# X-PLUG/Youku-mPLUG

Hardware: NVIDIA H100
Metric: video-text samples/sec (pretrain 1.3B, 8f x 224^2) (higher is better)
Workload: dtype bf16

## Files before the change

include/ymp.h:

```cpp
#ifndef YMP_H_
#define YMP_H_

#include <stddef.h>
#include <stdint.h>

#ifdef __cplusplus
extern "C" {
#endif

#define YMP_OK 0
#define YMP_EINVAL (-1)
#define YMP_ECUDA (-2)
#define YMP_ENOSUP (-3)

const char* ymp_last_error(void);
int ymp_abi_version(void);
uint64_t ymp_launch_count(void);
int ymp_set_pdl(int on);

typedef struct ymp_dropout_spec {
  const uint64_t* rng;
  uint32_t site;
  float p;
} ymp_dropout_spec;
// ... 110 lines not shown
  const void* k;
  const void* v;
  void* o;
  float* lse;
  int32_t ldq, ldk, ldv, ldo;
  int32_t q_head_stride, k_head_stride, v_head_stride, o_head_stride;
  ymp_seqmap map_q, map_kv, map_o;
  int32_t n_seq, n_heads, head_dim, s_q, s_kv;
  int32_t mask;
  int32_t mask_block;
  int64_t total_rows;
  float scale;
  ymp_dropout_spec drop;
  const int32_t* s_kv_dev;
  const int32_t* kv_rows;
  int64_t kv_rows_ld;
} ymp_attn_args;
int ymp_attn_fwd(const ymp_attn_args* a, void* stream);

typedef struct ymp_attn_prefix_table_args {
  ymp_attn_args attn;
  const int32_t* n_prefix;
} ymp_attn_prefix_table_args;
int ymp_attn_fwd_prefix_table(const ymp_attn_prefix_table_args* a, void* stream);

typedef struct ymp_attn_prefix_kv_args {
  ymp_attn_prefix_table_args table;
  const void* k_cache;
  const void* v_cache;
  int32_t ld_cache;
  int32_t cache_head_stride;
  int32_t n0;
  int32_t _pad;
} ymp_attn_prefix_kv_args;
int ymp_attn_fwd_prefix_kv(const ymp_attn_prefix_kv_args* a, void* stream);

typedef struct ymp_attn_bwd_args {
  ymp_attn_args fwd;
  const void* dout;
  void* dq;
  void* dk;
  void* dv;
  float* delta_ws;
  int32_t lddo, lddq, lddk, lddv;
  int32_t do_head_stride, dq_head_stride, dk_head_stride, dv_head_stride;
  ymp_seqmap map_do, map_dq, map_dkv;
} ymp_attn_bwd_args;
int ymp_attn_bwd(const ymp_attn_bwd_args* a, void* stream);
#define YMP_ATTN_PATH_MMA_SYNC 0
#define YMP_ATTN_PATH_WGMMA 1
#define YMP_ATTN_PATH_SMALL 2
#define YMP_ATTN_PATH_DECODE 3
int ymp_attn_last_path(void);

typedef struct ymp_im2col_args {
  const void* video;
  void* out;
  int32_t B, C, T, H, W, P, ldo;
} ymp_im2col_args;
int ymp_im2col(const ymp_im2col_args* a, void* stream);

typedef struct ymp_clip_args {
  const void* frames;
  void* out;
  const void* lut;
  int32_t B, T, H, W, C;
} ymp_clip_args;
int ymp_clip_normalize(const ymp_clip_args* a, void* stream);

typedef struct ymp_dropout_args {
  const void* x;
  void* y;
  int32_t rows, cols, ldx, ldy;
  int32_t dtype;
  int64_t row0;
  ymp_dropout_spec drop;
} ymp_dropout_args;
int ymp_dropout(const ymp_dropout_args* a, void* stream);

typedef struct ymp_embed_args {
  const int64_t* ids;
  const void* table;
  const void* pos;
  void* out;
  int32_t B, L, S, row_offset, hidden, vocab, ldo;
  int32_t out_dtype;
} ymp_embed_args;
int ymp_embed_gather(const ymp_embed_args* a, void* stream);

typedef struct ymp_ce_args {
  const void* logits;
  const int64_t* labels;
  float* loss;
  float* lse;
  const float* grad_rows;
  void* dlogits;
  int32_t rows, V, ld;
} ymp_ce_args;
int ymp_ce_fwd(const ymp_ce_args* a, void* stream);
int ymp_ce_bwd(const ymp_ce_args* a, void* stream);

typedef struct ymp_colsum_args {
  const void* in;
  float* out;
  int32_t R, C, ld;
} ymp_colsum_args;
// ... 34 lines not shown
```

youku-mplug_b200/csrc/attention.cu:

```cuda
#include <math_constants.h>
#include <stdlib.h>

#include "common.h"
#include "philox.cuh"
#include "ptx.cuh"
#include "wgmma.cuh"

namespace ymp {

struct SeqMap {
  int seq_div, n_prefix, prefix_per_seq;
  long outer_stride, inner_stride, pos_stride, prefix_base, prefix_stride;
};
static SeqMap to_map(const ymp_seqmap& m) {
  SeqMap r;
  r.seq_div = m.seq_div > 0 ? m.seq_div : 1;
  r.n_prefix = m.n_prefix; r.prefix_per_seq = m.prefix_per_seq;
  r.outer_stride = m.outer_stride; r.inner_stride = m.inner_stride; r.pos_stride = m.pos_stride;
  r.prefix_base = m.prefix_base; r.prefix_stride = m.prefix_stride;
  return r;
}
struct RSeq {
  long base, pos_stride, prefix0;
  int n_prefix;
// ... 293 lines not shown
  for (int r = 0; r < 2; ++r) {
    l_i[r] += __shfl_xor_sync(0xffffffffu, l_i[r], 1);
    l_i[r] += __shfl_xor_sync(0xffffffffu, l_i[r], 2);
  }
#pragma unroll
  for (int r = 0; r < 2; ++r) {
    const int qi = row_lo + g + r * 8;
    if ((unsigned)qi >= (unsigned)sq) continue;
    const float inv = l_i[r] > 0.f ? 1.f / l_i[r] : 0.f;
    __nv_bfloat16* orow = p.o + rrow(mo, qi) * p.ldo + h * p.hso;
#pragma unroll
    for (int nb = 0; nb < DIO / 8; ++nb)
      *reinterpret_cast<uint32_t*>(orow + nb * 8 + t4 * 2) = pack_bf16(o_acc[nb][2 * r] * inv, o_acc[nb][2 * r + 1] * inv);
    if (p.lse && t4 == 0) p.lse[((size_t)s * p.n_heads + h) * p.s_q + qi] = m_i[r] * p.scale + logf(l_i[r]);
  }
}
template <int D, int DIO>
__device__ __forceinline__ void store_dq(const AttnKParams& p, const float (&dq_acc)[D / 8][4], int row_lo, int sq, int h,
                                         const RSeq& mdq, int g, int t4) {
#pragma unroll
  for (int r = 0; r < 2; ++r) {
    const int qi = row_lo + g + r * 8;
    if (qi >= sq) continue;
    __nv_bfloat16* dqrow = p.dq + rrow(mdq, qi) * p.lddq + h * p.hsdq;
#pragma unroll
    for (int nb = 0; nb < DIO / 8; ++nb)
      *reinterpret_cast<uint32_t*>(dqrow + nb * 8 + t4 * 2) = pack_bf16(dq_acc[nb][2 * r] * p.scale, dq_acc[nb][2 * r + 1] * p.scale);
  }
}
template <int D, int DIO>
__device__ __forceinline__ void store_dkdv(const AttnKParams& p, const float (&dk_acc)[D / 8][4],
                                           const float (&dv_acc)[D / 8][4], int row_lo, int skv, int h, const RSeq& mdkv,
                                           int g, int t4) {
#pragma unroll
  for (int r = 0; r < 2; ++r) {
    const int kvr = row_lo + g + r * 8;
    if (kvr >= skv) continue;
    const long row = rrow(mdkv, kvr);
    __nv_bfloat16* dkrow = p.dk + row * p.lddk + h * p.hsdk;
    __nv_bfloat16* dvrow = p.dv + row * p.lddv + h * p.hsdv;
#pragma unroll
    for (int nb = 0; nb < DIO / 8; ++nb) {
      *reinterpret_cast<uint32_t*>(dkrow + nb * 8 + t4 * 2) = pack_bf16(dk_acc[nb][2 * r] * p.scale, dk_acc[nb][2 * r + 1] * p.scale);
      *reinterpret_cast<uint32_t*>(dvrow + nb * 8 + t4 * 2) = pack_bf16(dv_acc[nb][2 * r], dv_acc[nb][2 * r + 1]);
    }
  }
}

enum TileLayout {
  PADDED,
  SWIZZLE_128B
};
template <TileLayout L, int D, int DIO, class M>
__device__ __forceinline__ void load_tile(void* dst, const M& m, int r0, int n_valid, const int* rows = nullptr) {
  constexpr int CH = D / 8;
#pragma unroll
  for (int it = 0; it < (64 * CH + 127) / 128; ++it) {
    const int idx = threadIdx.x + it * 128;
    if ((64 * CH) % 128 != 0 && idx >= 64 * CH) break;
    const int r = idx / CH, c = idx - r * CH;
    uint8_t* d = L == PADDED ? reinterpret_cast<uint8_t*>(static_cast<__nv_bfloat16*>(dst) + r * (D + 8) + c * 8)
                             : static_cast<uint8_t*>(dst) + (c >> 3) * 8192 + r * 128 + (((c & 7) ^ (r & 7)) << 4);
    if ((unsigned)(r0 + r) < (unsigned)n_valid && (DIO == D || c * 8 < DIO))
      cp_async16(d, mrow(m, rows ? __ldg(rows + r0 + r) : r0 + r) + c * 8);
    else *reinterpret_cast<uint4*>(d) = make_uint4(0, 0, 0, 0);
  }
}

template <int D, int DIO>
__global__ void __launch_bounds__(128) attn_fwd_kernel(const AttnKParams p) {
  constexpr int LDS = D + 8, KS = D / 16, TILE = 64 * LDS;
  extern __shared__ __align__(16) uint8_t smem_attn[];
  __nv_bfloat16* Qs = reinterpret_cast<__nv_bfloat16*>(smem_attn);
  __nv_bfloat16* KVs = Qs + TILE;
  const int warp = threadIdx.x >> 5, lane = threadIdx.x & 31;
  const int q0 = blockIdx.x * 64, h = blockIdx.y, s = blockIdx.z;
  const int g = lane >> 2, t4 = lane & 3;
  griddep_launch();
  griddep_wait();
  int sq, skv;
  eff_len(p, s, sq, skv);
  if (q0 >= sq) return;
  const int* table = p.kv_rows ? p.kv_rows + s * p.kv_rows_ld : nullptr;
  const RSeq mkv = table ? RSeq{0, 1, 0, 0} : resolve(p.mkv, s), mo = resolve(p.mo, s);
  const RMat Mq = rmat(p.q, resolve(p.mq, s), p.ldq, h * p.hsq);
  const RMat Mk = rmat(p.k, mkv, p.ldk, h * p.hsk), Mv = rmat(p.v, mkv, p.ldv, h * p.hsv);
  int kv_begin;
  const int ntiles = key_tiles<true>(p, q0, sq, skv, kv_begin);

  load_tile<PADDED, D, DIO>(Qs, Mq, q0, sq);
  load_tile<PADDED, D, DIO>(KVs, Mk, kv_begin, skv, table);
  load_tile<PADDED, D, DIO>(KVs + TILE, Mv, kv_begin, skv, table);
  cp_async_commit();

  uint32_t qf[KS][4];
  float o_acc[D / 8][4];
#pragma unroll
  for (int i = 0; i < D / 8; ++i) { o_acc[i][0] = o_acc[i][1] = o_acc[i][2] = o_acc[i][3] = 0.f; }
  float m_i[2] = {-CUDART_INF_F, -CUDART_INF_F}, l_i[2] = {0.f, 0.f};
  const bool warp_active = (q0 + warp * 16) < sq;
  DropState ds;
  if (p.has_drop) ds = drop_state(p.drop);
  const uint32_t drow0 = (uint32_t)(((long)s * p.n_heads + h) * p.s_q + q0 + warp * 16 + g);

  for (int t = 0; t < ntiles; ++t) {
    const int kv0 = kv_begin + t * 64;
    __nv_bfloat16* Ks = KVs + (t & 1) * 2 * TILE;
    __nv_bfloat16* Vs = Ks + TILE;
    if (t + 1 < ntiles) {
      __nv_bfloat16* Kn = KVs + ((t + 1) & 1) * 2 * TILE;
      load_tile<PADDED, D, DIO>(Kn, Mk, kv0 + 64, skv, table);
      load_tile<PADDED, D, DIO>(Kn + TILE, Mv, kv0 + 64, skv, table);
      cp_async_commit();
      cp_async_wait<1>();
    } else {
      cp_async_wait<0>();
    }
    __syncthreads();
    if (t == 0) {
// ... 502 lines not shown
  const RSeq mkv = resolve(p.mkv, s), mdkv = resolve(p.mdkv, s);
  const RMat Mq = rmat(p.q, resolve(p.mq, s), p.ldq, h * p.hsq), Mdo = rmat(p.dout, resolve(p.mdo, s), p.lddo, h * p.hsdo);
  const RMat Mk = rmat(p.k, mkv, p.ldk, h * p.hsk), Mv = rmat(p.v, mkv, p.ldv, h * p.hsv);
  const int q_begin = (p.mask == MASK_CAUSAL) ? kv0 : 0;
  const int ntiles = (sq - q_begin + 63) / 64;
  const size_t stat_base = ((size_t)s * p.n_heads + h) * p.s_q;

  auto load_stage = [&](int stage, int qi0) {
    uint8_t* Qn = QDs + stage * 2 * TB;
    load_tile<SWIZZLE_128B, D, DIO>(Qn, Mq, qi0, sq);
    load_tile<SWIZZLE_128B, D, DIO>(Qn + TB, Mdo, qi0, sq);
    stage_dkdv_stats(p, stat_base, qi0, sq, stat + stage * 128);
  };

  load_tile<SWIZZLE_128B, D, DIO>(Ks, Mk, kv0, skv);
  load_tile<SWIZZLE_128B, D, DIO>(Vs, Mv, kv0, skv);
  load_stage(0, q_begin);
  cp_async_commit();

  float dk_acc[D / 8][4], dv_acc[D / 8][4];
#pragma unroll
  for (int i = 0; i < D / 8; ++i) {
    dk_acc[i][0] = dk_acc[i][1] = dk_acc[i][2] = dk_acc[i][3] = 0.f;
    dv_acc[i][0] = dv_acc[i][1] = dv_acc[i][2] = dv_acc[i][3] = 0.f;
  }
  DropState ds;
  if (p.has_drop) ds = drop_state(p.drop);
  const uint32_t dbase = (uint32_t)stat_base;

  for (int t = 0; t < ntiles; ++t) {
    const int qi0 = q_begin + t * 64;
    uint8_t* Qs = QDs + (t & 1) * 2 * TB;
    uint8_t* dOs = Qs + TB;
    const float* st = stat + (t & 1) * 128;
    if (t + 1 < ntiles) {
      load_stage((t + 1) & 1, qi0 + 64);
      cp_async_commit();
      cp_async_wait<1>();
    } else {
      cp_async_wait<0>();
    }
    fence_proxy_async();
    __syncthreads();
    float st_[8][4], dpt[8][4];
    wg_scores<D>(st_, smem_u32(Ks), smem_u32(Qs));
    wg_scores<D>(dpt, smem_u32(Vs), smem_u32(dOs));
    apply_mask_t<false>(p, st_, kv0 + warp * 16, qi0, skv, g, t4);
    probs_t<true>(p, ds, st_, dpt, st, dbase + (uint32_t)qi0, kv0 + warp * 16, lane);
    wg_pv<D>(dv_acc, st_, smem_u32(dOs));
    wg_pv<D>(dk_acc, dpt, smem_u32(Qs));
    __syncthreads();
  }
  store_dkdv<D, DIO>(p, dk_acc, dv_acc, kv0 + warp * 16, skv, h, mdkv, g, t4);
}

template <int D>
__global__ void __launch_bounds__(128) attn_decode_kernel(const AttnKParams p) {
  constexpr int CH = D / 8;
  extern __shared__ __align__(16) uint8_t smem_attn[];
  float (*o_part)[D + 1] = reinterpret_cast<float (*)[D + 1]>(smem_attn);
  float* l_part = reinterpret_cast<float*>(smem_attn) + 128 * (D + 1);
  float* m_part = l_part + 128;
  const int lane = threadIdx.x & 31, warp = threadIdx.x >> 5;
  const int h = blockIdx.x, s = blockIdx.y;
  griddep_launch();
  griddep_wait();
  const int* table = p.kv_rows ? p.kv_rows + s * p.kv_rows_ld : nullptr;
  const RSeq mkv = table ? RSeq{0, 1, 0, 0} : resolve(p.mkv, s);
  const RMat Mk = rmat(p.k, mkv, p.ldk, h * p.hsk), Mv = rmat(p.v, mkv, p.ldv, h * p.hsv);
  const __nv_bfloat16* qrow = p.q + rrow(resolve(p.mq, s), 0) * p.ldq + h * p.hsq;
  constexpr bool TWO_PHASE = D > 80;
  uint4 qv[CH], kv[CH], vv[CH];
#pragma unroll
  for (int c = 0; c < CH; ++c) qv[c] = __ldg(reinterpret_cast<const uint4*>(qrow) + c);
  auto row_of = [&](int key) { return table ? __ldg(table + key) : key; };
  auto fetch_k = [&](int row) {
    const uint4* kr = reinterpret_cast<const uint4*>(mrow(Mk, row));
#pragma unroll
    for (int c = 0; c < CH; ++c) kv[c] = __ldg(kr + c);
  };
  auto fetch_v = [&](int row) {
    const uint4* vr = reinterpret_cast<const uint4*>(mrow(Mv, row));
#pragma unroll
    for (int c = 0; c < CH; ++c) vv[c] = __ldg(vr + c);
  };
  if (warp * 32 + lane < p.s_kv) {
    const int row = row_of(warp * 32 + lane);
    fetch_k(row);
    if (!TWO_PHASE) fetch_v(row);
  }
  int sq, skv;
  eff_len(p, s, sq, skv);
  float o[D];
#pragma unroll
  for (int d = 0; d < D; ++d) o[d] = 0.f;
  float m_run = -CUDART_INF_F, l_run = 0.f;
  for (int k0 = 0; k0 < skv; k0 += 128) {
    const int key = k0 + warp * 32 + lane;
    const bool valid = key < skv;
    if (k0 > 0 && valid) {
      const int row = row_of(key);
      fetch_k(row);
      if (!TWO_PHASE) fetch_v(row);
    }
    float sc = -CUDART_INF_F;
    if (valid) {
// ... 40 lines not shown
  for (int r = 0; r < 128; ++r) l_all += l_part[r] * wgt[r >> 5];
  __nv_bfloat16* orow = p.o + rrow(resolve(p.mo, s), 0) * p.ldo + h * p.hso;
  for (int d = threadIdx.x; d < D; d += 128) {
    float acc = 0.f;
    for (int r = 0; r < 128; ++r) acc += o_part[r][d] * wgt[r >> 5];
    orow[d] = __float2bfloat16(acc / l_all);
  }
  if (p.lse && threadIdx.x == 0) p.lse[((long)s * p.n_heads + h) * p.s_q] = (m_all + log2f(l_all)) * 0.6931471805599453f;
}
static int fill_params(const ymp_attn_args* a, AttnKParams& p, const char* who) {
  YMP_CHECK_ARG(a && a->q && a->k && a->v, "%s: null q/k/v", who);
  YMP_CHECK_ARG(a->head_dim == 64 || a->head_dim == 80 || a->head_dim == 88 || a->head_dim == 96 || a->head_dim == 128,
                "%s: head_dim %d not in {64,80,88,96,128}", who, a->head_dim);
  YMP_CHECK_ARG(a->n_seq > 0 && a->n_heads > 0 && a->s_q > 0 && a->s_kv > 0, "%s: bad sizes", who);
  YMP_CHECK_ARG(a->ldq % 8 == 0 && a->ldk % 8 == 0 && a->ldv % 8 == 0 && a->ldo % 8 == 0, "%s: row strides must be multiples of 8", who);
  YMP_CHECK_ARG(a->q_head_stride % 8 == 0 && a->k_head_stride % 8 == 0 && a->v_head_stride % 8 == 0 && a->o_head_stride % 8 == 0, "%s: head strides must be multiples of 8", who);
  YMP_CHECK_ARG(aligned16(a->q) && aligned16(a->k) && aligned16(a->v), "%s: q/k/v must be 16-byte aligned", who);
  YMP_CHECK_ARG(a->mask >= 0 && a->mask <= 2, "%s: mask must be 0 (none), 1 (causal) or 2 (block-diagonal)", who);
  YMP_CHECK_ARG(a->mask == YMP_MASK_NONE || a->s_q == a->s_kv || (a->mask == YMP_MASK_CAUSAL && a->s_q < a->s_kv),
                "%s: block masks need s_q == s_kv, causal needs s_q <= s_kv", who);
  YMP_CHECK_ARG(a->mask != YMP_MASK_BLOCK || a->mask_block > 0, "%s: block mask needs mask_block > 0", who);
  YMP_CHECK_ARG(a->total_rows == 0 || (a->s_q == a->s_kv && a->total_rows > (int64_t)(a->n_seq - 1) * a->s_q),
                "%s: total_rows needs s_q == s_kv and must reach the last sequence", who);
  p.q = (const __nv_bfloat16*)a->q; p.k = (const __nv_bfloat16*)a->k; p.v = (const __nv_bfloat16*)a->v;
  p.o = (__nv_bfloat16*)a->o; p.lse = a->lse;
  p.ldq = a->ldq; p.ldk = a->ldk; p.ldv = a->ldv; p.ldo = a->ldo;
  p.hsq = a->q_head_stride; p.hsk = a->k_head_stride; p.hsv = a->v_head_stride; p.hso = a->o_head_stride;
  p.mq = to_map(a->map_q); p.mkv = to_map(a->map_kv); p.mo = to_map(a->map_o);
  p.n_seq = a->n_seq; p.n_heads = a->n_heads; p.s_q = a->s_q; p.s_kv = a->s_kv;
  p.mask = a->mask; p.mask_block = a->mask_block > 0 ? a->mask_block : 1; p.total_rows = a->total_rows;
  p.scale = a->scale; p.scale_log2 = a->scale * LOG2E;
  p.skv_dev = a->s_kv_dev;
  p.kv_rows = a->kv_rows; p.kv_rows_ld = a->kv_rows_ld;
  p.has_drop = (a->drop.rng && a->drop.p > 0.f) ? 1 : 0;
  p.drop.rng = (const uint64_t*)a->drop.rng; p.drop.site = a->drop.site; p.drop.p = a->drop.p;
  return YMP_OK;
}

template <int D_, int DIO_ = D_>
struct HeadDim {
  static constexpr int D = D_, DIO = DIO_;
};
template <bool WITH_128, class F>
static int for_head_dim(int head_dim, F&& launch) {
  switch (head_dim) {
    case 64: return launch(HeadDim<64>{});
    case 80: return launch(HeadDim<80>{});
    case 88: return launch(HeadDim<96, 88>{});
    case 96: return launch(HeadDim<96>{});
  }
  if constexpr (WITH_128) return launch(HeadDim<128>{});
  else return set_error(YMP_EINVAL, "attention: no kernel of this family for head_dim %d", head_dim);
}
template <void (*K)(AttnKParams), bool PDL>
static int launch_attn(dim3 grid, int smem, cudaStream_t st, const AttnKParams& p) {
  static DeviceOnce once;
  if (once.first()) { YMP_CUDA(cudaFuncSetAttribute(K, cudaFuncAttributeMaxDynamicSharedMemorySize, smem)); }
  if constexpr (PDL) launch_k(K, grid, dim3(128), smem, st, p);
  else K<<<grid, 128, smem, st>>>(p);
  YMP_LAUNCH_CHECK();
  return YMP_OK;
}

static int launch_decode(const AttnKParams& p, int head_dim, cudaStream_t st) {
  return for_head_dim<false>(head_dim, [&](auto hd) {
    constexpr int D = decltype(hd)::D;
    return launch_attn<attn_decode_kernel<D>, true>(dim3(p.n_heads, p.n_seq), (128 * (D + 1) + 128 + 4) * 4, st, p);
  });
}
static int launch_wg_fwd(const AttnKParams& p, int head_dim, cudaStream_t st) {
  const int lead = p.mask == MASK_CAUSAL ? (p.s_kv - p.s_q) & 63 : 0;
  const dim3 grid((p.s_q + lead + 63) / 64, p.n_heads, p.n_seq);
  return for_head_dim<false>(head_dim, [&](auto hd) {
    using H = decltype(hd);
    return launch_attn<attn_wg_fwd_kernel<H::D, H::DIO>, true>(grid, 5 * WgTile<H::D>::BYTES + 1024, st, p);
  });
}
template <bool CACHE>
static int launch_wg_fwd_table(const AttnKParams& p, int head_dim, cudaStream_t st) {
  const dim3 grid((p.s_q + 126) / 64, p.n_heads, p.n_seq);
  return for_head_dim<false>(head_dim, [&](auto hd) {
    using H = decltype(hd);
    return launch_attn<attn_wg_fwd_kernel<H::D, H::DIO, true, CACHE>, true>(grid, 5 * WgTile<H::D>::BYTES + 1024, st, p);
  });
}
static int launch_wg_bwd(const AttnKParams& p, int head_dim, cudaStream_t st) {
  return for_head_dim<false>(head_dim, [&](auto hd) {
    using H = decltype(hd);
    const int smem = 6 * WgTile<H::D>::BYTES + 1024 + 1024;
    const int rc = launch_attn<attn_wg_bwd_dq_kernel<H::D, H::DIO>, false>(dim3((p.s_q + 63) / 64, p.n_heads, p.n_seq), smem, st, p);
    if (rc) return rc;
    return launch_attn<attn_wg_bwd_dkdv_kernel<H::D, H::DIO>, false>(dim3((p.s_kv + 63) / 64, p.n_heads, p.n_seq), smem, st, p);
  });
}
static int launch_fwd(const AttnKParams& p, int head_dim, cudaStream_t st) {
  return for_head_dim<true>(head_dim, [&](auto hd) {
    using H = decltype(hd);
    return launch_attn<attn_fwd_kernel<H::D, H::DIO>, true>(dim3((p.s_q + 63) / 64, p.n_heads, p.n_seq), 5 * 64 * (H::D + 8) * 2, st, p);
  });
}
static int launch_bwd(const AttnKParams& p, int head_dim, cudaStream_t st) {
  return for_head_dim<true>(head_dim, [&](auto hd) {
    using H = decltype(hd);
    const int smem = 6 * 64 * (H::D + 8) * 2 + 1024;
    const int rc = launch_attn<attn_bwd_dq_kernel<H::D, H::DIO>, false>(dim3((p.s_q + 63) / 64, p.n_heads, p.n_seq), smem, st, p);
    if (rc) return rc;
    return launch_attn<attn_bwd_dkdv_kernel<H::D, H::DIO>, false>(dim3((p.s_kv + 63) / 64, p.n_heads, p.n_seq), smem, st, p);
  });
}

}

namespace ymp {
int attn_small_fwd_try(const ymp_attn_args* a, cudaStream_t st);
int attn_small_bwd_try(const ymp_attn_bwd_args* b, cudaStream_t st);
}

static thread_local int g_attn_path = -1;
extern "C" int ymp_attn_last_path(void) { return g_attn_path; }

extern "C" int ymp_attn_fwd(const ymp_attn_args* a, void* stream) {
  using namespace ymp;
  AttnKParams p = {};
  int rc = fill_params(a, p, "ymp_attn_fwd");
  if (rc) return rc;
  YMP_CHECK_ARG(a->o && aligned16(a->o), "ymp_attn_fwd: bad o");
  cudaStream_t st = (cudaStream_t)stream;
  const bool dropped = p.has_drop;
  YMP_CHECK_ARG(!dropped || a->drop.p < 1.f, "ymp_attn_fwd: dropout p must be < 1");
  if (a->kv_rows) {
    YMP_CHECK_ARG(a->s_q == 1 && a->mask == YMP_MASK_NONE && !dropped && a->total_rows == 0,
                  "ymp_attn_fwd: kv_rows needs s_q == 1, mask none, no dropout and no total_rows");
    YMP_CHECK_ARG(a->kv_rows_ld >= a->s_kv, "ymp_attn_fwd: kv_rows_ld must be >= s_kv");
  }
  if (a->mask == YMP_MASK_CAUSAL && a->s_q < a->s_kv) {
    YMP_CHECK_ARG(a->head_dim != 128, "ymp_attn_fwd: causal with s_q < s_kv needs head_dim 64, 80, 88 or 96");
    YMP_CHECK_ARG(!dropped, "ymp_attn_fwd: causal with s_q < s_kv takes no dropout");
    YMP_CHECK_ARG(!a->s_kv_dev, "ymp_attn_fwd: causal with s_q < s_kv takes no s_kv_dev");
    g_attn_path = YMP_ATTN_PATH_WGMMA;
    return launch_wg_fwd(p, a->head_dim, st);
  }
  if (a->s_q == 1 && a->mask == YMP_MASK_NONE && a->total_rows == 0 && !dropped && a->head_dim != 88 && a->head_dim != 128) {
    g_attn_path = YMP_ATTN_PATH_DECODE;
    return launch_decode(p, a->head_dim, st);
  }
  const bool dev_len = a->s_kv_dev != nullptr;
  YMP_CHECK_ARG(!dev_len || (!dropped && a->mask == YMP_MASK_NONE && a->total_rows == 0 && a->head_dim != 88),
                "ymp_attn_fwd: s_kv_dev needs mask none, no dropout, no total_rows, head_dim in {64,80,96,128}");
  if (!dropped && !dev_len && !a->kv_rows) {
    rc = attn_small_fwd_try(a, st);
    if (rc != YMP_ENOSUP) { g_attn_path = YMP_ATTN_PATH_SMALL; return rc; }
  }
  if (a->head_dim != 128 && a->mask != YMP_MASK_BLOCK && !dev_len && !a->kv_rows && !(a->s_q < 16 && a->s_kv > 256)) {
    g_attn_path = YMP_ATTN_PATH_WGMMA;
    return launch_wg_fwd(p, a->head_dim, st);
  }
  g_attn_path = YMP_ATTN_PATH_MMA_SYNC;
  return launch_fwd(p, a->head_dim, st);
}

static int fill_table_params(const ymp_attn_prefix_table_args* t, ymp::AttnKParams& p, const char* who) {
  using namespace ymp;
  YMP_CHECK_ARG(t->n_prefix != nullptr, "%s: null n_prefix table", who);
  const ymp_attn_args* a = &t->attn;
  int rc = fill_params(a, p, who);
  if (rc) return rc;
  YMP_CHECK_ARG(a->o && aligned16(a->o), "%s: bad o", who);
  YMP_CHECK_ARG(a->mask == YMP_MASK_CAUSAL, "%s: the mask must be causal", who);
  YMP_CHECK_ARG(a->head_dim != 128, "%s: needs head_dim 64, 80, 88 or 96", who);
  YMP_CHECK_ARG(!p.has_drop, "%s: takes no dropout", who);
  YMP_CHECK_ARG(a->total_rows == 0 && !a->s_kv_dev && !a->kv_rows, "%s: takes no total_rows, s_kv_dev or kv_rows", who);
  p.n_prefix = t->n_prefix;
  return YMP_OK;
}

extern "C" int ymp_attn_fwd_prefix_table(const ymp_attn_prefix_table_args* t, void* stream) {
  using namespace ymp;
  YMP_CHECK_ARG(t != nullptr, "ymp_attn_fwd_prefix_table: null args");
  AttnKParams p = {};
  const int rc = fill_table_params(t, p, "ymp_attn_fwd_prefix_table");
  if (rc) return rc;
  g_attn_path = YMP_ATTN_PATH_WGMMA;
  return launch_wg_fwd_table<false>(p, t->attn.head_dim, (cudaStream_t)stream);
}

extern "C" int ymp_attn_fwd_prefix_kv(const ymp_attn_prefix_kv_args* c, void* stream) {
  using namespace ymp;
  YMP_CHECK_ARG(c != nullptr, "ymp_attn_fwd_prefix_kv: null args");
  AttnKParams p = {};
  const int rc = fill_table_params(&c->table, p, "ymp_attn_fwd_prefix_kv");
  if (rc) return rc;
  YMP_CHECK_ARG(c->k_cache && c->v_cache && aligned16(c->k_cache) && aligned16(c->v_cache),
                "ymp_attn_fwd_prefix_kv: k_cache / v_cache must be non-null and 16-byte aligned");
  YMP_CHECK_ARG(c->ld_cache % 8 == 0 && c->cache_head_stride % 8 == 0,
                "ymp_attn_fwd_prefix_kv: ld_cache and cache_head_stride must be multiples of 8");
  YMP_CHECK_ARG(c->n0 >= 0, "ymp_attn_fwd_prefix_kv: n0 must be >= 0");
  p.kc = (const __nv_bfloat16*)c->k_cache; p.vc = (const __nv_bfloat16*)c->v_cache;
  p.ldc = c->ld_cache; p.hsc = c->cache_head_stride; p.n0 = c->n0;
  g_attn_path = YMP_ATTN_PATH_WGMMA;
  return launch_wg_fwd_table<true>(p, c->table.attn.head_dim, (cudaStream_t)stream);
}

extern "C" int ymp_attn_bwd(const ymp_attn_bwd_args* b, void* stream) {
  using namespace ymp;
  YMP_CHECK_ARG(b != nullptr, "ymp_attn_bwd: null args");
  const ymp_attn_args* a = &b->fwd;
  AttnKParams p = {};
  int rc = fill_params(a, p, "ymp_attn_bwd");
  if (rc) return rc;
  YMP_CHECK_ARG(a->o && a->lse && b->dout && b->dq && b->dk && b->dv && b->delta_ws, "ymp_attn_bwd: null o/lse/dout/dq/dk/dv/delta_ws");
  YMP_CHECK_ARG(b->lddo % 8 == 0 && b->lddq % 8 == 0 && b->lddk % 8 == 0 && b->lddv % 8 == 0, "ymp_attn_bwd: grad row strides must be multiples of 8");
  YMP_CHECK_ARG(!a->s_kv_dev, "ymp_attn_bwd: s_kv_dev is forward only");
  YMP_CHECK_ARG(!a->kv_rows, "ymp_attn_bwd: kv_rows is forward only");
  YMP_CHECK_ARG(a->mask != YMP_MASK_CAUSAL || a->s_q == a->s_kv, "ymp_attn_bwd: causal with s_q < s_kv is forward only");
  YMP_CHECK_ARG(!p.has_drop || a->drop.p < 1.f, "ymp_attn_bwd: dropout p must be < 1");
  p.dout = (const __nv_bfloat16*)b->dout; p.dq = (__nv_bfloat16*)b->dq; p.dk = (__nv_bfloat16*)b->dk; p.dv = (__nv_bfloat16*)b->dv;
  p.delta = b->delta_ws;
  p.lddo = b->lddo; p.hsdo = b->do_head_stride;
  p.lddq = b->lddq; p.lddk = b->lddk; p.lddv = b->lddv;
  p.hsdq = b->dq_head_stride; p.hsdk = b->dk_head_stride; p.hsdv = b->dv_head_stride;
  p.mdo = to_map(b->map_do); p.mdq = to_map(b->map_dq); p.mdkv = to_map(b->map_dkv);
  cudaStream_t st = (cudaStream_t)stream;
  if (!p.has_drop) {
    rc = attn_small_bwd_try(b, st);
    if (rc != YMP_ENOSUP) { g_attn_path = YMP_ATTN_PATH_SMALL; return rc; }
  }
  if (a->head_dim != 128 && a->mask != YMP_MASK_BLOCK) {
    g_attn_path = YMP_ATTN_PATH_WGMMA;
    return launch_wg_bwd(p, a->head_dim, st);
  }
  g_attn_path = YMP_ATTN_PATH_MMA_SYNC;
  return launch_bwd(p, a->head_dim, st);
}
```

youku-mplug_b200/ymp/lib.py:

```python
import ctypes as C
import os

_HERE = os.path.dirname(os.path.abspath(__file__))
LIB_PATH = os.path.join(_HERE, "libymp_b200.so")


class YmpError(RuntimeError):
    pass


if not os.path.exists(LIB_PATH):
    raise ImportError(
        f"{LIB_PATH} not found: build it with `make -C youku-mplug_b200/csrc` "
        "(or `python -c 'import __graft_entry__ as g; g.build()'`). There is no CPU fallback."
    )

lib = C.CDLL(LIB_PATH)

ACT_NONE, ACT_GELU_ERF, ACT_GELU_TANH = 0, 1, 2
MASK_NONE, MASK_CAUSAL, MASK_BLOCK = 0, 1, 2
DT_BF16, DT_F32 = 0, 1

c_i32 = C.c_int32
c_vp = C.c_void_p
# ... 79 lines not shown
        ("fwd", AttnArgs), ("dout", c_vp), ("dq", c_vp), ("dk", c_vp), ("dv", c_vp), ("delta_ws", c_vp),
        ("lddo", c_i32), ("lddq", c_i32), ("lddk", c_i32), ("lddv", c_i32),
        ("do_head_stride", c_i32), ("dq_head_stride", c_i32), ("dk_head_stride", c_i32), ("dv_head_stride", c_i32),
        ("map_do", SeqMap), ("map_dq", SeqMap), ("map_dkv", SeqMap),
    ]


class DropoutArgs(C.Structure):
    _fields_ = [("x", c_vp), ("y", c_vp), ("rows", c_i32), ("cols", c_i32), ("ldx", c_i32), ("ldy", c_i32),
                ("dtype", c_i32), ("row0", C.c_int64), ("drop", DropoutSpec)]


class Im2colArgs(C.Structure):
    _fields_ = [("video", c_vp), ("out", c_vp), ("B", c_i32), ("C", c_i32), ("T", c_i32), ("H", c_i32),
                ("W", c_i32), ("P", c_i32), ("ldo", c_i32)]


class ClipArgs(C.Structure):
    _fields_ = [("frames", c_vp), ("out", c_vp), ("lut", c_vp), ("B", c_i32), ("T", c_i32), ("H", c_i32), ("W", c_i32),
                ("C", c_i32)]


class EmbedArgs(C.Structure):
    _fields_ = [("ids", c_vp), ("table", c_vp), ("pos", c_vp), ("out", c_vp), ("B", c_i32), ("L", c_i32),
                ("S", c_i32), ("row_offset", c_i32), ("hidden", c_i32), ("vocab", c_i32), ("ldo", c_i32),
                ("out_dtype", c_i32)]


class CeArgs(C.Structure):
    _fields_ = [("logits", c_vp), ("labels", c_vp), ("loss", c_vp), ("lse", c_vp), ("grad_rows", c_vp),
                ("dlogits", c_vp), ("rows", c_i32), ("V", c_i32), ("ld", c_i32)]


class ColsumArgs(C.Structure):
    _fields_ = [("in_", c_vp), ("out", c_vp), ("R", c_i32), ("C", c_i32), ("ld", c_i32)]


class GroupArgs(C.Structure):
    _fields_ = [("in_", c_vp), ("out", c_vp), ("G", c_i32), ("T", c_i32), ("C", c_i32), ("ld_in", c_i32),
                ("ld_out", c_i32), ("broadcast", c_i32), ("scale", C.c_float)]


class AdamwArgs(C.Structure):
    _fields_ = [("master", c_vp), ("param", c_vp), ("grad", c_vp), ("m", c_vp), ("v", c_vp), ("sumsq", c_vp),
                ("n", C.c_int64), ("step", c_i32), ("lr", C.c_float), ("beta1", C.c_float), ("beta2", C.c_float),
                ("eps", C.c_float), ("weight_decay", C.c_float), ("grad_scale", C.c_float),
                ("max_grad_norm", C.c_float), ("hyper", c_vp), ("zero_grad", c_i32)]


lib.ymp_last_error.restype = C.c_char_p
lib.ymp_abi_version.restype = C.c_int
lib.ymp_launch_count.restype = C.c_uint64
lib.ymp_attn_last_path.restype = C.c_int
lib.ymp_set_pdl.restype = C.c_int
lib.ymp_set_pdl.argtypes = [C.c_int]
ATTN_PATH_MMA_SYNC, ATTN_PATH_WGMMA, ATTN_PATH_SMALL, ATTN_PATH_DECODE = 0, 1, 2, 3


def _declare(name, argstruct):
    fn = getattr(lib, name)
    fn.restype = C.c_int
    fn.argtypes = [C.POINTER(argstruct), c_vp]
    return fn


_gemm = _declare("ymp_gemm", GemmArgs)
_gemm_tiled = lib.ymp_gemm_tiled
_gemm_tiled.restype = C.c_int
_gemm_tiled.argtypes = [C.POINTER(GemmArgs), C.c_int, c_vp]
_gemm_skinny = _declare("ymp_gemm_skinny", GemmSkinnyArgs)
_gemm_skinny_wide = _declare("ymp_gemm_skinny_wide", GemmSkinnyArgs)
_ln_fwd = _declare("ymp_layernorm_fwd", LayerNormArgs)
_ln_bwd = _declare("ymp_layernorm_bwd", LayerNormBwdArgs)
_attn_fwd = _declare("ymp_attn_fwd", AttnArgs)
_attn_fwd_prefix_table = _declare("ymp_attn_fwd_prefix_table", AttnPrefixTableArgs)
_attn_fwd_prefix_kv = _declare("ymp_attn_fwd_prefix_kv", AttnPrefixKvArgs)
_attn_bwd = _declare("ymp_attn_bwd", AttnBwdArgs)
_im2col = _declare("ymp_im2col", Im2colArgs)
_clip = _declare("ymp_clip_normalize", ClipArgs)
_embed = _declare("ymp_embed_gather", EmbedArgs)
_ce_fwd = _declare("ymp_ce_fwd", CeArgs)
_ce_bwd = _declare("ymp_ce_bwd", CeArgs)
_colsum = _declare("ymp_colsum", ColsumArgs)
_group = _declare("ymp_group_reduce", GroupArgs)
_adamw = _declare("ymp_adamw", AdamwArgs)
_dropout = _declare("ymp_dropout", DropoutArgs)
_sumsq = lib.ymp_sumsq
_sumsq.restype = C.c_int
_sumsq.argtypes = [c_vp, C.c_int64, c_vp, c_vp]


def check(rc, what):
    if rc != 0:
        raise YmpError(f"{what} failed ({rc}): {lib.ymp_last_error().decode()}")


def launch_count():
    return int(lib.ymp_launch_count())


def set_pdl(on):
    return int(lib.ymp_set_pdl(int(bool(on))))


def attn_last_path():
    return int(lib.ymp_attn_last_path())


def ptr(t):
    return None if t is None else t.data_ptr()


def cur_stream():
    import torch
    return torch.cuda.current_stream().cuda_stream


def call(fn, args, what):
    check(fn(C.byref(args), cur_stream()), what)
```

Baseline: 167.4.

## Add one-CTA-per-head short-sequence attention kernels keeping whole K/V in smem

```diff
diff --git a/include/ymp.h b/include/ymp.h
--- a/include/ymp.h
+++ b/include/ymp.h
@@ -186,6 +186,7 @@
 #define YMP_ATTN_PATH_SMALL 2
 #define YMP_ATTN_PATH_DECODE 3
 int ymp_attn_last_path(void);
+int ymp_attn_last_short(void);
 
 typedef struct ymp_im2col_args {
   const void* video;
diff --git a/youku-mplug_b200/csrc/attention.cu b/youku-mplug_b200/csrc/attention.cu
--- a/youku-mplug_b200/csrc/attention.cu
+++ b/youku-mplug_b200/csrc/attention.cu
@@ -369,11 +369,11 @@
   SWIZZLE_128B
 };
 template <TileLayout L, int D, int DIO, class M>
-__device__ __forceinline__ void load_tile(void* dst, const M& m, int r0, int n_valid, const int* rows = nullptr) {
+__device__ __forceinline__ void load_tile_by(int tid, void* dst, const M& m, int r0, int n_valid, const int* rows = nullptr) {
   constexpr int CH = D / 8;
 #pragma unroll
   for (int it = 0; it < (64 * CH + 127) / 128; ++it) {
-    const int idx = threadIdx.x + it * 128;
+    const int idx = tid + it * 128;
     if ((64 * CH) % 128 != 0 && idx >= 64 * CH) break;
     const int r = idx / CH, c = idx - r * CH;
     uint8_t* d = L == PADDED ? reinterpret_cast<uint8_t*>(static_cast<__nv_bfloat16*>(dst) + r * (D + 8) + c * 8)
@@ -382,6 +382,10 @@
       cp_async16(d, mrow(m, rows ? __ldg(rows + r0 + r) : r0 + r) + c * 8);
     else *reinterpret_cast<uint4*>(d) = make_uint4(0, 0, 0, 0);
   }
+}
+template <TileLayout L, int D, int DIO, class M>
+__device__ __forceinline__ void load_tile(void* dst, const M& m, int r0, int n_valid, const int* rows = nullptr) {
+  load_tile_by<L, D, DIO>(threadIdx.x, dst, m, r0, n_valid, rows);
 }
 
 template <int D, int DIO>
@@ -990,6 +994,236 @@
     __syncthreads();
   }
   store_dkdv<D, DIO>(p, dk_acc, dv_acc, kv0 + warp * 16, skv, h, mdkv, g, t4);
+}
+
+constexpr int SHORT_MAX = 256, SHORT_THREADS = 256, SHORT_TILES = SHORT_MAX / 64;
+
+__device__ __forceinline__ void wg_bar(int wg) { asm volatile("bar.sync %0, 128;" ::"r"(1 + wg) : "memory"); }
+
+template <int D, int DIO>
+__global__ void __launch_bounds__(SHORT_THREADS, 1) attn_short_fwd_kernel(const AttnKParams p) {
+  constexpr int TB = WgTile<D>::BYTES;
+  extern __shared__ uint8_t smem_wg[];
+  uint8_t* sm = smem_wg + ((1024u - (smem_u32(smem_wg) & 1023u)) & 1023u);
+  uint8_t* Qs = sm;
+  uint8_t* Ks = sm + SHORT_TILES * TB;
+  uint8_t* Vs = sm + 2 * SHORT_TILES * TB;
+  const int wg = threadIdx.x >> 7, tid = threadIdx.x & 127, warp = tid >> 5, lane = threadIdx.x & 31;
+  const int h = blockIdx.y, s = blockIdx.z;
+  const int g = lane >> 2, t4 = lane & 3;
+  griddep_launch();
+  griddep_wait();
+  int sq, skv;
+  eff_len(p, s, sq, skv);
+  if (sq <= 0) return;
+  const int nq = (sq + 63) / 64, nk = (skv + 63) / 64;
+  const RSeq mkv = resolve(p.mkv, s), mo = resolve(p.mo, s);
+  const RMat Mq = rmat(p.q, resolve(p.mq, s), p.ldq, h * p.hsq);
+  const RMat Mk = rmat(p.k, mkv, p.ldk, h * p.hsk), Mv = rmat(p.v, mkv, p.ldv, h * p.hsv);
+  for (int i = wg; i < nq; i += 2) load_tile_by<SWIZZLE_128B, D, DIO>(tid, Qs + i * TB, Mq, i * 64, sq);
+  if (wg == 0) {
+    load_tile_by<SWIZZLE_128B, D, DIO>(tid, Ks, Mk, 0, skv);
+    load_tile_by<SWIZZLE_128B, D, DIO>(tid, Vs, Mv, 0, skv);
+  }
+  cp_async_commit();
+  for (int i = 2 - wg; i < nk; i += 2) {
+    load_tile_by<SWIZZLE_128B, D, DIO>(tid, Ks + i * TB, Mk, i * 64, skv);
+    load_tile_by<SWIZZLE_128B, D, DIO>(tid, Vs + i * TB, Mv, i * 64, skv);
+  }
+  cp_async_commit();
+  cp_async_wait<1>();
+  fence_proxy_async();
+  __syncthreads();
+
+  for (int pass = 0; pass < 2; ++pass) {
+    const int qt = pass == 0 ? wg : 3 - wg, q0 = qt * 64;
+    const bool active = qt < nq;
+    if (pass == 1 && !active) break;
+    float o_acc[D / 8][4];
+#pragma unroll
+    for (int i = 0; i < D / 8; ++i) { o_acc[i][0] = o_acc[i][1] = o_acc[i][2] = o_acc[i][3] = 0.f; }
+    float m_i[2] = {-CUDART_INF_F, -CUDART_INF_F}, l_i[2] = {0.f, 0.f};
+    for (int t = 0; t < nk; ++t) {
+      if (pass == 0 && t == 1) {
+        cp_async_wait<0>();
+        fence_proxy_async();
+        __syncthreads();
+      }
+      if (!active) continue;
+      const int kv0 = t * 64;
+      float sc[8][4];
+      wg_scores<D>(sc, smem_u32(Qs + qt * TB), smem_u32(Ks + t * TB));
+      if (tile_needs_mask(p, q0 + warp * 16, kv0, skv)) apply_mask(p, sc, q0 + warp * 16, kv0, skv, g, t4, -CUDART_INF_F);
+      softmax_step(p, sc, m_i, l_i, o_acc);
+      wg_pv<D>(o_acc, sc, smem_u32(Vs + t * TB));
+    }
+    if (active) store_o_lse<D, DIO>(p, o_acc, m_i, l_i, q0 + warp * 16, sq, s, h, mo, g, t4);
+  }
+}
+
+template <int D, int DIO>
+__global__ void __launch_bounds__(SHORT_THREADS, 1) attn_short_bwd_dq_kernel(const AttnKParams p) {
+  constexpr int TB = WgTile<D>::BYTES;
+  extern __shared__ uint8_t smem_wg[];
+  uint8_t* sm = smem_wg + ((1024u - (smem_u32(smem_wg) & 1023u)) & 1023u);
+  uint8_t* Ks = sm;
+  uint8_t* Vs = sm + SHORT_TILES * TB;
+  const int wg = threadIdx.x >> 7, tid = threadIdx.x & 127, warp = tid >> 5, lane = threadIdx.x & 31;
+  uint8_t* Qs = sm + (2 * SHORT_TILES + 2 * wg) * TB;
+  uint8_t* dOs = Qs + TB;
+  float* stat = reinterpret_cast<float*>(sm + (2 * SHORT_TILES + 4) * TB) + wg * 128;
+  const int h = blockIdx.y, s = blockIdx.z;
+  const int g = lane >> 2, t4 = lane & 3;
+  int sq, skv;
+  eff_len(p, s, sq, skv);
+  if (sq <= 0) return;
+  const int nq = (sq + 63) / 64, nk = (skv + 63) / 64;
+  const RSeq mkv = resolve(p.mkv, s), mo = resolve(p.mo, s), mdo = resolve(p.mdo, s), mdq = resolve(p.mdq, s);
+  const RMat Mq = rmat(p.q, resolve(p.mq, s), p.ldq, h * p.hsq), Mdo = rmat(p.dout, mdo, p.lddo, h * p.hsdo);
+  const RMat Mk = rmat(p.k, mkv, p.ldk, h * p.hsk), Mv = rmat(p.v, mkv, p.ldv, h * p.hsv);
+  if (wg < nq) {
+    load_tile_by<SWIZZLE_128B, D, DIO>(tid, Qs, Mq, wg * 64, sq);
+    load_tile_by<SWIZZLE_128B, D, DIO>(tid, dOs, Mdo, wg * 64, sq);
+  }
+  if (wg == 0) {
+    load_tile_by<SWIZZLE_128B, D, DIO>(tid, Ks, Mk, 0, skv);
+    load_tile_by<SWIZZLE_128B, D, DIO>(tid, Vs, Mv, 0, skv);
+  }
+  cp_async_commit();
+  for (int i = 2 - wg; i < nk; i += 2) {
+    load_tile_by<SWIZZLE_128B, D, DIO>(tid, Ks + i * TB, Mk, i * 64, skv);
+    load_tile_by<SWIZZLE_128B, D, DIO>(tid, Vs + i * TB, Mv, i * 64, skv);
+  }
+  cp_async_commit();
+  if (wg < nq) stage_dq_stats<DIO>(p, s, h, wg * 64 + warp * 16, sq, mo, mdo, stat + warp * 16);
+  cp_async_wait<1>();
+  fence_proxy_async();
+  __syncthreads();
+
+  for (int pass = 0; pass < 2; ++pass) {
+    const int qt = pass == 0 ? wg : 3 - wg, q0 = qt * 64;
+    const bool active = qt < nq;
+    if (pass == 1 && !active) break;
+    if (pass == 1) {
+      wg_bar(wg);
+      load_tile_by<SWIZZLE_128B, D, DIO>(tid, Qs, Mq, q0, sq);
+      load_tile_by<SWIZZLE_128B, D, DIO>(tid, dOs, Mdo, q0, sq);
+      cp_async_commit();
+      stage_dq_stats<DIO>(p, s, h, q0 + warp * 16, sq, mo, mdo, stat + warp * 16);
+      cp_async_wait<0>();
+      fence_proxy_async();
+      wg_bar(wg);
+    }
+    float lse_r[2] = {0.f, 0.f}, del_r[2] = {0.f, 0.f};
+    if (active) {
+      lse_r[0] = stat[warp * 16 + g]; lse_r[1] = stat[warp * 16 + g + 8];
+      del_r[0] = stat[64 + warp * 16 + g]; del_r[1] = stat[64 + warp * 16 + g + 8];
+    }
+    float dq_acc[D / 8][4];
+#pragma unroll
+    for (int i = 0; i < D / 8; ++i) { dq_acc[i][0] = dq_acc[i][1] = dq_acc[i][2] = dq_acc[i][3] = 0.f; }
+    for (int t = 0; t < nk; ++t) {
+      if (pass == 0 && t == 1) {
+        cp_async_wait<0>();
+        fence_proxy_async();
+        __syncthreads();
+      }
+      if (!active) continue;
+      const int kv0 = t * 64;
+      float sc[8][4], dp[8][4];
+      wg_scores<D>(sc, smem_u32(Qs), smem_u32(Ks + t * TB));
+      wg_scores<D>(dp, smem_u32(dOs), smem_u32(Vs + t * TB));
+      if (tile_needs_mask(p, q0 + warp * 16, kv0, skv)) apply_mask(p, sc, q0 + warp * 16, kv0, skv, g, t4, -CUDART_INF_F);
+      scores_to_ds(p, sc, dp, lse_r, del_r);
+      wg_pv<D>(dq_acc, sc, smem_u32(Ks + t * TB));
+    }
+    if (active) store_dq<D, DIO>(p, dq_acc, q0 + warp * 16, sq, h, mdq, g, t4);
+  }
+}
+
+template <int D, int DIO>
+__global__ void __launch_bounds__(SHORT_THREADS, 1) attn_short_bwd_dkdv_kernel(const AttnKParams p) {
+  constexpr int TB = WgTile<D>::BYTES;
+  extern __shared__ uint8_t smem_wg[];
+  uint8_t* sm = smem_wg + ((1024u - (smem_u32(smem_wg) & 1023u)) & 1023u);
+  uint8_t* Qs = sm;
+  uint8_t* dOs = sm + SHORT_TILES * TB;
+  const int wg = threadIdx.x >> 7, tid = threadIdx.x & 127, warp = tid >> 5, lane = threadIdx.x & 31;
+  uint8_t* Ks = sm + (2 * SHORT_TILES + 2 * wg) * TB;
+  uint8_t* Vs = Ks + TB;
+  float* stat = reinterpret_cast<float*>(sm + (2 * SHORT_TILES + 4) * TB);
+  const int h = blockIdx.y, s = blockIdx.z;
+  const int g = lane >> 2, t4 = lane & 3;
+  int sq, skv;
+  eff_len(p, s, sq, skv);
+  if (skv <= 0) return;
+  const int nq = (sq + 63) / 64, nk = (skv + 63) / 64;
+  const RSeq mkv = resolve(p.mkv, s), mdkv = resolve(p.mdkv, s);
+  const RMat Mq = rmat(p.q, resolve(p.mq, s), p.ldq, h * p.hsq), Mdo = rmat(p.dout, resolve(p.mdo, s), p.lddo, h * p.hsdo);
+  const RMat Mk = rmat(p.k, mkv, p.ldk, h * p.hsk), Mv = rmat(p.v, mkv, p.ldv, h * p.hsv);
+  const size_t stat_base = ((size_t)s * p.n_heads + h) * p.s_q;
+  if (wg < nk) {
+    load_tile_by<SWIZZLE_128B, D, DIO>(tid, Ks, Mk, wg * 64, skv);
+    load_tile_by<SWIZZLE_128B, D, DIO>(tid, Vs, Mv, wg * 64, skv);
+  }
+  if (wg == 0) {
+    load_tile_by<SWIZZLE_128B, D, DIO>(tid, Qs, Mq, 0, sq);
+    load_tile_by<SWIZZLE_128B, D, DIO>(tid, dOs, Mdo, 0, sq);
+  }
+  cp_async_commit();
+  for (int i = 2 - wg; i < nq; i += 2) {
+    load_tile_by<SWIZZLE_128B, D, DIO>(tid, Qs + i * TB, Mq, i * 64, sq);
+    load_tile_by<SWIZZLE_128B, D, DIO>(tid, dOs + i * TB, Mdo, i * 64, sq);
+  }
+  cp_async_commit();
+  for (int i = threadIdx.x; i < nq * 64; i += SHORT_THREADS) {
+    float* st = stat + (i >> 6) * 128 + (i & 63);
+    st[0] = i < sq ? p.lse[stat_base + i] * LOG2E : CUDART_INF_F;
+    st[64] = i < sq ? p.delta[stat_base + i] : 0.f;
+  }
+  cp_async_wait<1>();
+  fence_proxy_async();
+  __syncthreads();
+  DropState ds;
+  const uint32_t dbase = (uint32_t)stat_base;
+
+  for (int pass = 0; pass < 2; ++pass) {
+    const int kt = pass == 0 ? wg : 3 - wg, kv0 = kt * 64;
+    const bool active = kt < nk;
+    if (pass == 1 && !active) break;
+    if (pass == 1) {
+      wg_bar(wg);
+      load_tile_by<SWIZZLE_128B, D, DIO>(tid, Ks, Mk, kv0, skv);
+      load_tile_by<SWIZZLE_128B, D, DIO>(tid, Vs, Mv, kv0, skv);
+      cp_async_commit();
+      cp_async_wait<0>();
+      fence_proxy_async();
+      wg_bar(wg);
+    }
+    float dk_acc[D / 8][4], dv_acc[D / 8][4];
+#pragma unroll
+    for (int i = 0; i < D / 8; ++i) {
+      dk_acc[i][0] = dk_acc[i][1] = dk_acc[i][2] = dk_acc[i][3] = 0.f;
+      dv_acc[i][0] = dv_acc[i][1] = dv_acc[i][2] = dv_acc[i][3] = 0.f;
+    }
+    for (int t = 0; t < nq; ++t) {
+      if (pass == 0 && t == 1) {
+        cp_async_wait<0>();
+        fence_proxy_async();
+        __syncthreads();
+      }
+      if (!active) continue;
+      const int qi0 = t * 64;
+      float st_[8][4], dpt[8][4];
+      wg_scores<D>(st_, smem_u32(Ks), smem_u32(Qs + t * TB));
+      wg_scores<D>(dpt, smem_u32(Vs), smem_u32(dOs + t * TB));
+      apply_mask_t<false>(p, st_, kv0 + warp * 16, qi0, skv, g, t4);
+      probs_t<true>(p, ds, st_, dpt, stat + t * 128, dbase + (uint32_t)qi0, kv0 + warp * 16, lane);
+      wg_pv<D>(dv_acc, st_, smem_u32(dOs + t * TB));
+      wg_pv<D>(dk_acc, dpt, smem_u32(Qs + t * TB));
+    }
+    if (active) store_dkdv<D, DIO>(p, dk_acc, dv_acc, kv0 + warp * 16, skv, h, mdkv, g, t4);
+  }
 }
 
 template <int D>
@@ -1136,12 +1370,12 @@
   if constexpr (WITH_128) return launch(HeadDim<128>{});
   else return set_error(YMP_EINVAL, "attention: no kernel of this family for head_dim %d", head_dim);
 }
-template <void (*K)(AttnKParams), bool PDL>
+template <void (*K)(AttnKParams), bool PDL, int THREADS = 128>
 static int launch_attn(dim3 grid, int smem, cudaStream_t st, const AttnKParams& p) {
   static DeviceOnce once;
   if (once.first()) { YMP_CUDA(cudaFuncSetAttribute(K, cudaFuncAttributeMaxDynamicSharedMemorySize, smem)); }
-  if constexpr (PDL) launch_k(K, grid, dim3(128), smem, st, p);
-  else K<<<grid, 128, smem, st>>>(p);
+  if constexpr (PDL) launch_k(K, grid, dim3(THREADS), smem, st, p);
+  else K<<<grid, THREADS, smem, st>>>(p);
   YMP_LAUNCH_CHECK();
   return YMP_OK;
 }
@@ -1177,6 +1411,23 @@
     return launch_attn<attn_wg_bwd_dkdv_kernel<H::D, H::DIO>, false>(dim3((p.s_kv + 63) / 64, p.n_heads, p.n_seq), smem, st, p);
   });
 }
+static int launch_short_fwd(const AttnKParams& p, int head_dim, cudaStream_t st) {
+  return for_head_dim<false>(head_dim, [&](auto hd) {
+    using H = decltype(hd);
+    const int smem = 3 * SHORT_TILES * WgTile<H::D>::BYTES + 1024;
+    return launch_attn<attn_short_fwd_kernel<H::D, H::DIO>, true, SHORT_THREADS>(dim3(1, p.n_heads, p.n_seq), smem, st, p);
+  });
+}
+static int launch_short_bwd(const AttnKParams& p, int head_dim, cudaStream_t st) {
+  return for_head_dim<false>(head_dim, [&](auto hd) {
+    using H = decltype(hd);
+    const dim3 grid(1, p.n_heads, p.n_seq);
+    const int tiles = (2 * SHORT_TILES + 4) * WgTile<H::D>::BYTES + 1024;
+    const int rc = launch_attn<attn_short_bwd_dq_kernel<H::D, H::DIO>, false, SHORT_THREADS>(grid, tiles + 2 * 128 * 4, st, p);
+    if (rc) return rc;
+    return launch_attn<attn_short_bwd_dkdv_kernel<H::D, H::DIO>, false, SHORT_THREADS>(grid, tiles + SHORT_TILES * 128 * 4, st, p);
+  });
+}
 static int launch_fwd(const AttnKParams& p, int head_dim, cudaStream_t st) {
   return for_head_dim<true>(head_dim, [&](auto hd) {
     using H = decltype(hd);
@@ -1201,7 +1452,14 @@
 }
 
 static thread_local int g_attn_path = -1;
+static thread_local int g_attn_short = 0;
 extern "C" int ymp_attn_last_path(void) { return g_attn_path; }
+extern "C" int ymp_attn_last_short(void) { return g_attn_short; }
+
+static bool short_seq(const ymp_attn_args* a, bool dropped) {
+  return a->mask == YMP_MASK_NONE && !dropped && a->s_q <= ymp::SHORT_MAX && a->s_kv <= ymp::SHORT_MAX &&
+         (a->head_dim == 64 || a->head_dim == 80 || a->head_dim == 96) && !a->s_kv_dev && !a->kv_rows;
+}
 
 extern "C" int ymp_attn_fwd(const ymp_attn_args* a, void* stream) {
   using namespace ymp;
@@ -1211,6 +1469,7 @@
   YMP_CHECK_ARG(a->o && aligned16(a->o), "ymp_attn_fwd: bad o");
   cudaStream_t st = (cudaStream_t)stream;
   const bool dropped = p.has_drop;
+  g_attn_short = 0;
   YMP_CHECK_ARG(!dropped || a->drop.p < 1.f, "ymp_attn_fwd: dropout p must be < 1");
   if (a->kv_rows) {
     YMP_CHECK_ARG(a->s_q == 1 && a->mask == YMP_MASK_NONE && !dropped && a->total_rows == 0,
@@ -1237,6 +1496,10 @@
   }
   if (a->head_dim != 128 && a->mask != YMP_MASK_BLOCK && !dev_len && !a->kv_rows && !(a->s_q < 16 && a->s_kv > 256)) {
     g_attn_path = YMP_ATTN_PATH_WGMMA;
+    if (short_seq(a, dropped)) {
+      g_attn_short = 1;
+      return launch_short_fwd(p, a->head_dim, st);
+    }
     return launch_wg_fwd(p, a->head_dim, st);
   }
   g_attn_path = YMP_ATTN_PATH_MMA_SYNC;
@@ -1261,6 +1524,7 @@
 extern "C" int ymp_attn_fwd_prefix_table(const ymp_attn_prefix_table_args* t, void* stream) {
   using namespace ymp;
   YMP_CHECK_ARG(t != nullptr, "ymp_attn_fwd_prefix_table: null args");
+  g_attn_short = 0;
   AttnKParams p = {};
   const int rc = fill_table_params(t, p, "ymp_attn_fwd_prefix_table");
   if (rc) return rc;
@@ -1271,6 +1535,7 @@
 extern "C" int ymp_attn_fwd_prefix_kv(const ymp_attn_prefix_kv_args* c, void* stream) {
   using namespace ymp;
   YMP_CHECK_ARG(c != nullptr, "ymp_attn_fwd_prefix_kv: null args");
+  g_attn_short = 0;
   AttnKParams p = {};
   const int rc = fill_table_params(&c->table, p, "ymp_attn_fwd_prefix_kv");
   if (rc) return rc;
@@ -1288,6 +1553,7 @@
 extern "C" int ymp_attn_bwd(const ymp_attn_bwd_args* b, void* stream) {
   using namespace ymp;
   YMP_CHECK_ARG(b != nullptr, "ymp_attn_bwd: null args");
+  g_attn_short = 0;
   const ymp_attn_args* a = &b->fwd;
   AttnKParams p = {};
   int rc = fill_params(a, p, "ymp_attn_bwd");
@@ -1311,6 +1577,10 @@
   }
   if (a->head_dim != 128 && a->mask != YMP_MASK_BLOCK) {
     g_attn_path = YMP_ATTN_PATH_WGMMA;
+    if (short_seq(a, p.has_drop)) {
+      g_attn_short = 1;
+      return launch_short_bwd(p, a->head_dim, st);
+    }
     return launch_wg_bwd(p, a->head_dim, st);
   }
   g_attn_path = YMP_ATTN_PATH_MMA_SYNC;
diff --git a/youku-mplug_b200/ymp/lib.py b/youku-mplug_b200/ymp/lib.py
--- a/youku-mplug_b200/ymp/lib.py
+++ b/youku-mplug_b200/ymp/lib.py
@@ -155,6 +155,7 @@
 lib.ymp_abi_version.restype = C.c_int
 lib.ymp_launch_count.restype = C.c_uint64
 lib.ymp_attn_last_path.restype = C.c_int
+lib.ymp_attn_last_short.restype = C.c_int
 lib.ymp_set_pdl.restype = C.c_int
 lib.ymp_set_pdl.argtypes = [C.c_int]
 ATTN_PATH_MMA_SYNC, ATTN_PATH_WGMMA, ATTN_PATH_SMALL, ATTN_PATH_DECODE = 0, 1, 2, 3
@@ -210,6 +211,10 @@
     return int(lib.ymp_attn_last_path())
 
 
+def attn_last_short():
+    return bool(lib.ymp_attn_last_short())
+
+
 def ptr(t):
     return None if t is None else t.data_ptr()
 
```

After: 169.7, median of 6. 1.01x the previous value.
